# KumarRobotics/top_down_renderer

Measured on AMD Instinct MI355X. Metric: particle-updates/sec (render+score+resample), higher is better.
Workload: dtype f32

## Files before the change

include/tdr.h:

```cpp
#ifndef TDR_H_
#define TDR_H_

#include <stddef.h>
#include <stdint.h>

#ifdef __cplusplus
extern "C" {
#endif

#define TDR_OK 0
#define TDR_ERR_ARG (-1)
#define TDR_ERR_HIP (-2)
#define TDR_ERR_NOMEM (-3)

#define TDR_MAX_CLASSES 15
#define TDR_ST_FIELDS 7
enum { TDR_ST_INIT_X = 0, TDR_ST_INIT_Y = 1, TDR_ST_DX = 2, TDR_ST_DY = 3, TDR_ST_THETA = 4, TDR_ST_SCALE = 5,
       TDR_ST_HAVE_INIT = 6 };

typedef struct tdr_state {
  float init_x_px, init_y_px, dx_m, dy_m, theta, scale;
  uint8_t have_init;
  uint8_t pad_[3];
} tdr_state;
// ... 190 lines not shown
int tdr_config_compact(int on);
int tdr_config_shift_uniform(int mode);
float tdr_config_shift_uniform_span(float cells);
int tdr_config_ray_split(int k);
int tdr_config_cart_skip(int on);
int tdr_config_init_mfma(int on);
int tdr_config_uw_waves(int on);
int64_t tdr_shift_uniform_launches(void);

int tdr_profile_enable(int on);
int tdr_profile_score_ms(double* total_ms, int64_t* launches);
int tdr_profile_shares(double* dense_ms, double* scattered_ms, int64_t* scattered_particles);
int tdr_profile_variants(int64_t out[16]);

int64_t tdr_config_tuning(const char* name, int64_t value);
int tdr_selftest_score(void);
int tdr_k_selftest_round(const float* x, int64_t n, float limit, int32_t* out, void* stream);
int tdr_libm_variant(void);
int tdr_libm_force_variant(int variant);
int tdr_sincosf_host(const float* x, int64_t n, int variant, float* sin_out, float* cos_out);
int tdr_k_selftest_sincos(const float* x, int64_t n, float* sin_out, float* cos_out, void* stream);
int tdr_logf_host(const float* x, int64_t n, float* out);
int tdr_k_selftest_logf(const float* x, int64_t n, float* out, void* stream);
int tdr_k_selftest_atan2(const float* y, const float* x, int64_t n, float* out, void* stream);

int tdr_k_states_aos_to_soa(const tdr_state* aos, int64_t n, float* st, int64_t cap, void* stream);
int tdr_k_states_soa_to_aos(const float* st, int64_t cap, int64_t n, tdr_state* aos, void* stream);
size_t tdr_locality_tmp_ints(int64_t n, int map_rows, int map_cols);
int tdr_k_locality_order(const float* st, int64_t cap, int64_t n, int map_rows, int map_cols, int32_t* perm_out,
                         int32_t* keys_tmp, void* stream);
// ... 162 lines not shown
```

top_down_renderer_amd/_lib.py:

```python
import ctypes as C
import os

_PKG = os.path.dirname(os.path.abspath(__file__))
SO_PATH = os.environ.get("TDR_LIB_PATH") or os.path.join(_PKG, "libtdr_hip.so")

TDR_ST_FIELDS = 7
TDR_MAX_CLASSES = 15
TDR_SVG_NO_KEY = 0xFFFFFFFF


class FilterParamsC(C.Structure):
    _fields_ = [
        ("pos_cov", C.c_float), ("theta_cov", C.c_float), ("regularization", C.c_float),
        ("init_pos_px_x", C.c_float), ("init_pos_px_y", C.c_float), ("init_pos_px_cov", C.c_float),
        ("init_pos_m_x", C.c_float), ("init_pos_m_y", C.c_float),
        ("init_pos_deg_theta", C.c_float), ("init_pos_deg_cov", C.c_float),
        ("force_on_map", C.c_int32),
        ("fixed_scale", C.c_float), ("scale_log_min", C.c_float), ("scale_log_max", C.c_float),
        ("num_classes", C.c_int32),
        ("class_weights", C.c_float * 16),
    ]


class MapDescC(C.Structure):
# ... 96 lines not shown
    "tdr_rng_pipe_from_host": (_i, [_vp, _vp, _vp]),
    "tdr_rng_pipe_to_host": (_i, [_vp, _vp, _vp]),
    "tdr_rng_pipe_normals": (_i, [_vp, _i64, _i64, _i64, _i, C.POINTER(_vp), _vp]),
    "tdr_rng_pipe_uniform": (_i, [_vp, C.POINTER(_vp), _vp]),
    "tdr_rng_dev_workspace_bytes": (C.c_size_t, [_i64]),
    "tdr_k_rng_propagate_normals": (_i, [_vp, _i64, _i64, _i64, _i, _vp, _vp, _vp]),
    "tdr_k_rng_uniform": (_i, [_vp, _vp, _vp]),
    "tdr_rng_get_state_host": (_i, [_vp, _vp]),
    "tdr_rng_set_state_host": (_i, [_vp, _vp]),
    "tdr_k_resample_dev": (_i, [_vp, _i64, _i64, _vp, _i64, _i64, _vp, _vp]),
    "tdr_score_ctx_create": (_i, [C.POINTER(_vp)]),
    "tdr_score_ctx_destroy": (None, [_vp]),
    "tdr_score_ctx_span": (C.c_float, [_vp]),
    "tdr_score_ctx_trial_calls": (_i64, [_vp]),
    "tdr_config_tuning": (_i64, [C.c_char_p, _i64]),
    "tdr_selftest_score": (_i, []),
    "tdr_profile_variants": (_i, [C.POINTER(_i64)]),
    "tdr_score_ctx_set_polar_factors": (_i, [_vp, _vp, _i, _i]),
    "tdr_polar_factors_host": (_i, [_i, _i, _f, _f, _vp]),
    "tdr_k_score_polar_ctx": (_i, [C.POINTER(MapDescC), _vp, _vp, _i, _i, _f, C.POINTER(FilterParamsC), _vp, _i64, _i64,
                                   _i64, _vp, _f, _i, _vp, _vp, _vp, _vp]),
    "tdr_score_geo_workspace_floats": (C.c_size_t, [_i, _i, _i, _i64, _i64]),
    "tdr_k_score_polar_geo": (_i, [C.POINTER(MapDescC), C.POINTER(MapDescC), _vp, _vp, _vp, _f, _f, _i, _i, _f,
                                   C.POINTER(FilterParamsC), _vp, _i64, _i64, _i64, _vp, _f, _i, _vp, _vp, _vp]),
    "tdr_score_cart_workspace_floats": (C.c_size_t, [_i, _i, _i, _i64, _i64]),
    "tdr_k_score_cart": (_i, [C.POINTER(MapDescC), _vp, _i, _i, _f, C.POINTER(FilterParamsC), _vp, _i64, _i64, _i64,
                              _vp, _vp, _vp, _vp]),
    "tdr_score_cart_init_workspace_floats": (C.c_size_t, [_i, _i, _i, _i64, _i64]),
    "tdr_k_score_cart_init": (_i, [C.POINTER(MapDescC), _vp, _i, _i, _f, C.POINTER(FilterParamsC), _vp, _i64, _i64, _i64,
                                   _vp, _vp]),
# ... 141 lines not shown
```

top_down_renderer_amd/csrc/tdr_score.hip:

```cpp

#include "tdr_common.h"
#include "tdr_batch.h"
#include "tdr_sincosf.h"

struct ScoreArgs {
  const float* rec;
  int rows, cols;
  float resolution;
  const float* tab;
  const float* utab = nullptr;
  const float* scan_pk;
  int nb, nr;
  float res;
  const float* st;
  int64_t cap, n;
  const int32_t* order;
  const int32_t* count = nullptr;
  const int32_t* slot_base = nullptr;
  int use_theta_override = 0;
  float theta_override = 0.f;
  int only_uninit = 0;
  int group, nchunks;
  int64_t npad;
  float* part;
  const uint32_t* crec = nullptr;
  const float* dict = nullptr;
  int dict_n = 0;
  int ctiles_r = 0;
  unsigned kmask_off = 0;
  int kmask_row = 0;
  const int32_t* run_if = nullptr;
};

#include "tdr_score_dev.h"
#include "tdr_score_init.h"
#include "tdr_score_su.h"
#include "tdr_score_cart.h"


#ifdef TDR_SCORE_TIMELINE
#define TDR_TL_MAX (1 << 17)
__device__ unsigned long long g_timeline[2 * TDR_TL_MAX];
extern "C" int tdr_debug_read_timeline(unsigned long long* out, int n) {
  return hipMemcpyFromSymbol(out, HIP_SYMBOL(g_timeline), sizeof(unsigned long long) * 2 * (size_t)n) == hipSuccess ? 0 : -1;
}
#endif
template <int NV4, int U, bool KSLOT, bool USCALE, bool COMPACT, bool WIDE = false>
__device__ __forceinline__ void score_polar_body(const ScoreArgs& a, const unsigned bx, const unsigned by) {
  constexpr int RF = 4 * NV4;
  static_assert(!WIDE || (COMPACT && NV4 == 2), "wide compact records: 8-float dense records only");
  constexpr int CW = WIDE ? 4 : CmapShape<RF, KSLOT>::CW, LC = WIDE ? 1 : CmapShape<RF, KSLOT>::LC;
  constexpr int NDICT = WIDE ? TDR_CMAP_WIDE_MAX_DICT : TDR_CMAP_MAX_DICT;
#ifdef TDR_SCORE_TIMELINE
  const unsigned tl_id = blockIdx.y * gridDim.x + blockIdx.x;
  if (threadIdx.x == 0 && tl_id < TDR_TL_MAX) g_timeline[2 * tl_id] = wall_clock64();
#endif
  extern __shared__ float4 ring[];
  __shared__ float ldict[COMPACT ? NDICT : 1];
  const int lane = threadIdx.x & 63, wave = threadIdx.x >> 6;
  const int64_t slot = ((int64_t)bx * 4 + wave) * 64 + lane;
  if (a.run_if && !int_form_off(a.run_if)) return;
  const int64_t nact = a.count ? (int64_t)*a.count : a.n;
  if ((int64_t)bx * 256 >= nact) return;
  const bool valid = slot < nact;
  const int64_t sbase = a.slot_base ? (int64_t)*a.slot_base : 0;
  const int64_t p = a.order ? (int64_t)a.order[sbase + (valid ? slot : 0)] : (valid ? slot : 0);
  if (a.only_uninit && !__syncthreads_or(valid && a.st[TDR_ST_HAVE_INIT * a.cap + p] == 0.f)) return;
  const float scale = a.st[TDR_ST_SCALE * a.cap + p];
  const float cx = a.st[TDR_ST_DX * a.cap + p] * scale + a.st[TDR_ST_INIT_X * a.cap + p];
  const float cy = a.st[TDR_ST_DY * a.cap + p] * scale + a.st[TDR_ST_INIT_Y * a.cap + p];
  const float off0 = cy / a.resolution;
// ... 142 lines not shown
          int row = ic + shift;
          row -= row >= nb ? nb : 0;
          boff[u] = cell_offset(tab_at((int64_t)(j0 + jj) * nb + ic));
          sp[u] = rj + __mul24(row, rs);
        }
        step(std::false_type{}, boff, sp, min(U, nb - i));
      }
    }
  }
  if (sbase + slot < a.npad) {
    float* o = a.part + (int64_t)by * (RF + 1) * a.npad + sbase + slot;
#pragma unroll
    for (int k = 0; k < RF; k++) o[(int64_t)k * a.npad] = acc[k];
    o[(int64_t)RF * a.npad] = KSLOT ? acc[RF - 2] : known;
  }
#ifdef TDR_SCORE_TIMELINE
  __syncthreads();
  if (threadIdx.x == 0 && tl_id < TDR_TL_MAX) g_timeline[2 * tl_id + 1] = wall_clock64();
#endif
}
template <int NV4, int U, bool KSLOT, bool USCALE, bool COMPACT, bool WIDE = false>
__global__ __launch_bounds__(256, COMPACT ? (WIDE ? 3 : 5) : 1) void score_polar_kernel(ScoreArgs a) {
#if TDR_XCD_SWIZZLE
  const unsigned nbx = gridDim.x, per = (nbx + 7) / 8;
  unsigned bx = (blockIdx.x % 8) * per + blockIdx.x / 8;
  if (nbx % 8 != 0) bx = blockIdx.x;
#else
  const unsigned bx = blockIdx.x;
#endif
  score_polar_body<NV4, U, KSLOT, USCALE, COMPACT, WIDE>(a, bx, blockIdx.y);
}
template <int NV4, int U, bool KSLOT, bool USCALE, bool COMPACT, bool WIDE = false>
__global__ __launch_bounds__(256, COMPACT ? (WIDE ? 3 : 5) : 1) void score_polar_batch_kernel(const ScoreArgs* __restrict__ args,
                                                                                              const int32_t* __restrict__ blk, int k) {
// ... 396 lines not shown
#define TDR_CART_WAVE_MUL 2
static int64_t g_score_waves = 131072;
static int g_score_group = 0;
static int g_su_group = 0;
static int64_t score_wave_target() { return g_score_waves; }
extern "C" int tdr_config_init_ahead(int);
extern "C" int tdr_config_batch_init_search(int);
extern "C" int tdr_config_prefix_head(int);
extern "C" int tdr_config_ray_block_major(int);
extern "C" int tdr_config_ray_patch(int);
extern "C" int tdr_config_ray_borrow(int);
extern "C" int tdr_config_cart_seg_rows(int);
extern "C" int tdr_config_mt_stretches(int);
extern "C" int tdr_config_su_wave_span(int);
extern "C" int tdr_config_su_lds_pad(int);
extern "C" int tdr_config_init_device(int);
extern "C" int64_t tdr_config_init_window_words(int64_t);
extern "C" int64_t tdr_config_cart_init_chunk(int64_t);
extern "C" int64_t tdr_config_tuning(const char* name, int64_t value) {
  if (!name) return -1;
  const std::string n(name);
  if (n == "score_waves") { if (value > 0) g_score_waves = value; return g_score_waves; }
  if (n == "score_group") { if (value >= 0) g_score_group = (int)value; return g_score_group; }
  if (n == "su_group") { if (value >= 0) g_su_group = (int)value; return g_su_group; }
  if (n == "batch_init_search") return tdr_config_batch_init_search((int)std::max<int64_t>(value, -1));
  if (n == "init_ahead") return tdr_config_init_ahead((int)std::min<int64_t>(std::max<int64_t>(value, -1), 3));
  if (n == "prefix_head") return tdr_config_prefix_head((int)std::max<int64_t>(value, -1));
  if (n == "ray_borrow") return tdr_config_ray_borrow((int)std::max<int64_t>(value, -1));
  if (n == "ray_patch") return tdr_config_ray_patch((int)std::max<int64_t>(value, -1));
  if (n == "ray_block_major") return tdr_config_ray_block_major((int)std::max<int64_t>(value, -1));
  if (n == "cart_seg_rows") return tdr_config_cart_seg_rows((int)std::max<int64_t>(value, -1));
  if (n == "mt_stretches") return tdr_config_mt_stretches((int)std::max<int64_t>(value, -1));
  if (n == "su_lds_pad") return tdr_config_su_lds_pad((int)std::max<int64_t>(value, -1));
  if (n == "su_wave_span") return tdr_config_su_wave_span((int)std::max<int64_t>(value, -1));
  if (n == "init_device") return tdr_config_init_device((int)std::max<int64_t>(value, -1));
  if (n == "init_window_words") return tdr_config_init_window_words(value > 0 ? value : -1);
  if (n == "cart_init_chunk") return tdr_config_cart_init_chunk(value > 0 ? value : -1);
  return -1;
}
static void choose_chunks(int64_t n, int nr, int& rpc, int& nchunks, int target_mul = 1) {
  int64_t nbatches = cdiv(std::max<int64_t>(n, 1), 64);
  int64_t want = std::max<int64_t>(1, cdiv(score_wave_target() * target_mul, nbatches));
  nchunks = (int)std::min<int64_t>(nr, want);
  rpc = (int)cdiv(nr, nchunks);
  nchunks = (int)cdiv(nr, rpc);
}

__global__ void utab_kernel(const float* __restrict__ tab, int64_t n2, float scale, float res,
// ... 5 lines not shown
static int score_group_rings(int nb, int nr, int rf, int64_t n_total) {
  const int forced = g_score_group;
  const int64_t ring_bytes = std::max<int64_t>((int64_t)nb * rf * 4, 1);
  int g = (int)std::min<int64_t>(8, (32 * 1024) / ring_bytes);
  const int64_t chunks_wanted = cdiv(2048, cdiv(std::max<int64_t>(n_total, 1), 256));
  g = (int)std::min<int64_t>(g, std::max<int64_t>(1, nr / std::max<int64_t>(chunks_wanted, 1)));
  if (forced > 0) g = forced;
  g = std::max(1, std::min<int>(g, (int)((60 * 1024) / ring_bytes)));
  if (g >= TDR_SCORE_U) g -= g % TDR_SCORE_U;
  return std::max(g, 1);
}
extern "C" int tdr_cmap_words(int ncls);
struct ScoreWs {
  int group, nchunks;
  int su_group, su_nchunks;
  int64_t npad, npad_part, off_aux, off_utab, off_su, total;
  bool su;
  SuWs suw;
};
static ScoreWs score_ws(int ncls, int nb, int nr, int64_t n, int64_t n_total) {
  ScoreWs w;
  const int rf = tdr_rec_floats(ncls);
  if (n_total <= 0) n_total = n;
  w.group = score_group_rings(nb, nr, rf, n_total);
  if (w.group % 4 != 0 && tdr_cmap_words(ncls) != 0 && tdr_su_shape_ok(nb, nr, 4, n_total))
    w.group = std::max(4, w.group - w.group % 4);
  w.nchunks = (int)cdiv(nr, w.group);
  w.npad = cdiv(std::max<int64_t>(n, 1), 64) * 64;
  w.su = tdr_su_shape_ok(nb, nr, w.group, n_total) && tdr_cmap_words(ncls) != 0;
  w.su_group = w.group;
  {
    const int forced = g_su_group;
    if (w.su && w.group == 4 && nr % 8 == 0 && cdiv(n_total, 256) * (nr / 8) >= 4096) w.su_group = 8;
    if (w.su && forced >= 4 && forced % 4 == 0) w.su_group = forced;
  }
  w.su_nchunks = (int)cdiv(nr, w.su_group);
  w.npad_part = w.su ? su_npad(std::max<int64_t>(n, 1), nb) : w.npad;
  w.off_aux = w.su ? (int64_t)std::max(std::max(w.nchunks, w.su_nchunks), TDR_RAY_MAX_SPLIT) * std::max(rf + 1, 2 * ncls + 2) * w.npad_part
                   : (int64_t)w.nchunks * (rf + 1) * w.npad_part;
  w.off_utab = w.off_aux + 3 * w.npad + 64;
  w.off_su = (w.off_utab + 2 * (int64_t)nb * nr + 63) / 64 * 64;
  w.total = w.off_su;
  if (w.su) {
    w.suw = tdr_su_ws(nb, nr, w.su_group, std::max<int64_t>(n, 1));
    w.total += w.suw.total;
  }
  return w;
}
extern "C" size_t tdr_score_workspace_floats(int ncls, int nb, int nr, int64_t n, int64_t n_total) {
  if (ncls < 1 || ncls > TDR_MAX_CLASSES || nb < 1 || nr < 1 || n < 0) return 0;
  return (size_t)score_ws(ncls, nb, nr, n, n_total).total;
}
static int fill_utab(ScoreArgs& a, float* workspace, const ScoreWs& W, float uniform_scale, hipStream_t s) {
// ... 405 lines not shown
  a.part = workspace;
  int rc = fill_utab(a, workspace, W, uniform_scale, s);
  if (rc) return rc;
  float* res_flag = workspace + W.off_aux;
  if (init_search)
    if ((rc = tdr_score_init_search(map, a.tab, a.utab, scan_pk, nb, nr, res, fp, st, cap, n, n_total, perm, res_flag, a.npad, s)))
      return rc;
  FinalizeArgs f = make_finalize_args(map, fp, a.part, a.nchunks, a.npad, (int64_t)nb * nr, st, cap, n, perm, raw_w);
  if (int_form_applies(W, map, rf)) {
    const int32_t* slots = nullptr;
    const int32_t* counts = nullptr;
    SuLaunch L;
    L.map = map; L.tab = a.utab ? a.utab : a.tab; L.uniform_scale = a.utab != nullptr; L.scan_pk = scan_pk;
    L.nb = nb; L.nr = nr; L.rf = rf; L.res = res; L.st = st; L.cap = cap; L.n = n; L.perm = perm;
    L.group = W.su_group; L.nchunks = W.su_nchunks; L.npad = W.npad_part; L.part = a.part;
    L.fac = ctx && ctx->fac && ctx->fac_nb == nb && ctx->fac_nr == nr ? ctx->fac : nullptr;
    L.uscale = uniform_scale;
    L.wave_span = tdr_su_wave_span();
    L.ray_split = tdr_ray_splits(nb, nr, n, tdr_ray_block_major(L));
    L.ws = reinterpret_cast<int32_t*>(workspace + W.off_su);
    TunerScope tuner_scope(ctx, s);
    L.span = tdr_su_span_begin(ctx ? &ctx->tuner : nullptr,
                               ((int64_t)n << 24) ^ ((int64_t)nb << 12) ^ nr ^ ((int64_t)map->rows << 40), s);
    if ((rc = tdr_su_prepare(L, W.suw, s, &slots, &counts))) return rc;
    if ((rc = tdr_ray_prepare(L, W.suw, s))) return rc;
    const int32_t* inexact = counts + 4;
    {
      ScoreProfScope prof(s);
      {
        ShareProfScope sp(0, s, true);
        if ((rc = tdr_ray_score(L, W.suw, s))) return rc;
      }
      {
        ShareProfScope sp(1, s, true);
        if ((rc = tdr_su_score(L, W.suw, s))) return rc;
      }
      if (g_prof_on) { g_share_valid = true; g_share_counts = counts; }
      ScoreArgs r = a;
      r.run_if = inexact;
      if ((rc = launch_score(r, map, rf, s, false))) return rc;
    }
    launch_finalize_exact(f, map, W.npad_part, slots, counts, inexact, W.su_nchunks, L.ray_split, s);
    LAUNCH_CHECK("score_finalize_exact");
    launch_finalize(f, n, s);
  } else {
    if ((rc = launch_score(a, map, rf, s))) return rc;
    launch_finalize(f, n, s);
  }
  LAUNCH_CHECK("score_finalize");
  if (init_search) return tdr_score_init_fixup(res_flag, n, fp->regularization, raw_w, s);
  return TDR_OK;
}

__global__ void init_from_best_kernel(const float* __restrict__ best_cost, const float* __restrict__ best_theta,
                                      const int32_t* __restrict__ order, int64_t n, float* __restrict__ st, int64_t cap,
                                      GateArgs gate, float* __restrict__ res_flag) {
  const int64_t slot = (int64_t)blockIdx.x * blockDim.x + threadIdx.x;
// ... 166 lines not shown
```

top_down_renderer_amd/csrc/tdr_score_dev.h:

```cpp
#ifndef TDR_SCORE_DEV_H_
#define TDR_SCORE_DEV_H_
#include "tdr_common.h"

__device__ __forceinline__ int rot_shift_dev(float rot, int nb) {
  int s = (int)round((double)(rot * (float)nb / 2) / M_PI);
  s %= nb;
  if (s < 0) s += nb;
  return s;
}

__device__ __forceinline__ int round_half_away_clamped(float x) {
  const float y = x + 0.49999997f;
  int r;
  asm("v_cvt_flr_i32_f32 %0, %1" : "=v"(r) : "v"(y));
  return r;
}

template <int RF, bool KSLOT>
struct CmapShape {
  static constexpr int ND = KSLOT ? RF - 2 : RF - 1;
  static constexpr int CW = (ND + 2) / 3 <= 1 ? 1 : ((ND + 2) / 3 == 2 ? 2 : 4);
  static constexpr int LC = CW == 1 ? 3 : (CW == 2 ? 2 : 1);
};
template <int CW, int LC>
// ... 83 lines not shown
}

template <int RF, bool KSLOT>
__device__ __forceinline__ void cmap_decode_wide(const uint32_t (&w)[4], const float* ldict, float (&m)[RF]) {
  constexpr int ND = CmapShape<RF, KSLOT>::ND;
  static_assert(ND <= 7, "wide records hold up to seven distances");
#pragma unroll
  for (int k = 0; k < ND; k++) {
    const uint32_t boff = (k & 1) ? (w[k / 2] >> 16) : (w[k / 2] & 0xFFFCu);
    m[k] = *reinterpret_cast<const float*>(reinterpret_cast<const char*>(ldict) + boff);
  }
  const float kf = (float)(w[3] & 1u);
  if (KSLOT) m[RF - 2] = kf;
  m[RF - 1] = kf;
}
#endif
```

top_down_renderer_amd/csrc/tdr_score_ray.hip:

```cpp
#include "tdr_score_dev.h"
#include "tdr_score_su.h"

#define RAY_PR 16
#define RAY_PG 16
#define RAY_PATCH_MAX_NB 256
static bool g_ray_borrow = true;
extern "C" int tdr_config_ray_borrow(int on) {
  if (on >= 0) g_ray_borrow = on != 0;
  return g_ray_borrow ? 1 : 0;
}
static bool g_ray_patch = true;
extern "C" int tdr_config_ray_patch(int on) {
  if (on >= 0) g_ray_patch = on != 0;
  return g_ray_patch ? 1 : 0;
}
static bool g_ray_bm = true;
extern "C" int tdr_config_ray_block_major(int on) {
  if (on >= 0) g_ray_bm = on != 0;
  return g_ray_bm ? 1 : 0;
}
static inline bool ray_bm(const SuLaunch& L) { return g_ray_bm && L.fac != nullptr; }
static inline bool ray_patch(const SuLaunch& L) { return ray_bm(L) && g_ray_patch && L.nb % RAY_PG == 0 && L.nb <= RAY_PATCH_MAX_NB; }
static inline int ray_gq(int nr, bool bm) { return bm ? 1 : (nr <= 64 ? 1 : (nr <= 128 ? 2 : 4)); }
static inline int ray_blocks(int nr, bool bm) { return (int)cdiv(nr, 64 * ray_gq(nr, bm)); }
// ... 348 lines not shown
    if (lane == 0) {
      o[(int64_t)(2 * c) * a.npad] = (uint32_t)s;
      o[(int64_t)(2 * c + 1) * a.npad] = (uint32_t)(s >> 32);
    }
  }
#pragma unroll
  for (int dlt = 32; dlt > 0; dlt >>= 1) {
    known += __shfl_xor(known, dlt, 64);
    norm += __shfl_xor(norm, dlt, 64);
  }
  if (lane == 0) {
    o[(int64_t)(2 * a.ncls) * a.npad] = norm;
    o[(int64_t)(2 * a.ncls + 1) * a.npad] = known;
  }
}
template <int GQ, bool USCALE, bool BM = false, bool PATCH = false>
__global__ __launch_bounds__(256) void score_polar_ray_kernel(RayArgs a) {
  extern __shared__ unsigned long long lacc[];
  __shared__ uint32_t ldict[TDR_CMAP_MAX_DICT];
  __shared__ uint4 lut[16];
  __shared__ float2 ldir[PATCH ? RAY_PATCH_MAX_NB : 1];
  if (int_form_off(a.inexact)) return;
  if (a.fac && a.inexact[2] == 0) ray_body<GQ, USCALE, true, BM, PATCH>(a, lacc, ldict, lut, ldir);
  else ray_body<GQ, USCALE, false, BM, PATCH>(a, lacc, ldict, lut, ldir);
}


extern "C" size_t tdr_cmap_plane_offset_words(int ncls, int rows, int cols);
extern "C" size_t tdr_cmap_plane_words(int ncls, int rows, int cols);

bool tdr_ray_map_ok(const tdr_map_desc* map) {
  return map->crec && map->dict && map->cwords == tdr_cmap_words(map->ncls) && map->dict_n > 0 &&
         map->dict_n <= TDR_CMAP_MAX_DICT && tdr_cmap_plane_words(map->ncls, map->rows, map->cols) != 0;
}
static int g_ray_split = 0;
extern "C" int tdr_config_ray_split(int k) {
  if (k >= 0) g_ray_split = k > TDR_RAY_MAX_SPLIT ? TDR_RAY_MAX_SPLIT : k;
  return g_ray_split;
}
// ... 80 lines not shown
```

top_down_renderer_amd/csrc/tdr_score_su.h:

```cpp
#ifndef TDR_SCORE_SU_H_
#define TDR_SCORE_SU_H_
#include "tdr_common.h"

static inline int64_t su_npad(int64_t n, int nb) { return cdiv(n + 63 * std::min<int64_t>(nb, n), 64) * 64; }
bool tdr_su_shape_ok(int nb, int nr, int group, int64_t n_total);
struct SuWs {
  int64_t tab_su, desc, bbox, keys_in, keys_out, vals_in, vals_out, ints, slots, sort_tmp, ray_tab, ray_desc, ray_multi, ray_rad, total;
  int64_t slots2, wave_tmp;
};
#define TDR_SU_TAIL_INTS 10
#define TDR_RAY_MAX_SPLIT 8
SuWs tdr_su_ws(int nb, int nr, int group, int64_t n);

struct SuLaunch {
  const tdr_map_desc* map;
  const float* tab;
  bool uniform_scale;
  const float* scan_pk;
  int nb, nr, rf;
  float res;
  const float* st;
  int64_t cap, n;
  const int32_t* perm;
  int group, nchunks;
  int64_t npad;
  float* part;
  int ray_split;
  const float* fac;
  float uscale;
  int32_t* ws;
  float span;
  float wave_span = 0.f;
};
int tdr_su_prepare(const SuLaunch& L, const SuWs& W, hipStream_t s, const int32_t** slots_out, const int32_t** counts_out);
int tdr_su_order(const SuLaunch& L, const SuWs& W, hipStream_t s, const int32_t** slots_out, const int32_t** counts_out);
struct SpanTuner {
  int64_t shape = -1;
  int phase = -2;
  int settled_launches = 0;
// ... 19 lines not shown
```

top_down_renderer_amd/csrc/tdr_score_su.hip:

```cpp
#include <rocprim/device/device_radix_sort.hpp>

#include <atomic>

#include "tdr_score_dev.h"
#include "tdr_score_su.h"
#include "tdr_score_su_asm.h"

#define SU_CODE_FULL 0xFFu
#define SU_CODE_FULL_ALL 0xFEu
#define SU_CODE_PAD 0xFDu
#define SU_NSECT 8
#define SU_BOX_WORDS 4096

struct SuArgs {
  const uint32_t* crec;
  const uint32_t* kmask;
  int kcolw;
  unsigned kmask_off;
  const uint32_t* dict_int;
  int dict_n, ctiles_r;
  int pkcol;
  const int32_t* inexact;
  int rows, cols;
  float resolution;
  const float* tab_su;
  const uint32_t* desc;
  const float* bbox;
  const float* scan_pk;
  int nb, nr;
  float res;
  const float* st;
  int64_t cap;
  const int32_t* slots;
  const int32_t* nslots;
  int group, nchunks, ncls;
  int64_t npad;
  uint32_t* part;
  uint32_t* stats;
};

__global__ __launch_bounds__(256) void su_prep_kernel(const float* __restrict__ tab, const float* __restrict__ scan_pk,
                                                      int nb, int nr, int rf, int ncls, int ckconst, unsigned pbase,
                                                      unsigned plane_bytes, int group, int nchunks,
                                                      const float* __restrict__ dict, int dict_n, float* __restrict__ tab_su,
                                                      uint32_t* __restrict__ desc) {
  const int64_t t = (int64_t)blockIdx.x * blockDim.x + threadIdx.x;
  bool bad = false;
  for (int k = threadIdx.x; k < dict_n; k += blockDim.x) bad |= !(fabsf(dict[k]) <= 3.402823466e+38f);
  const bool dict_bad = __syncthreads_or(bad);
  const int64_t total = (int64_t)nchunks * nb * group;
// ... 228 lines not shown
    const int rank = __popcll(valid & (((uint64_t)1 << (t & 63)) - 1));
    out[(int64_t)counts[0] + oc1 + moved[w] + rank] = p;
  }
}
__global__ void su_copy_slots_kernel(const int32_t* __restrict__ src, const int32_t* __restrict__ counts, int32_t* __restrict__ dst) {
  const int64_t t = (int64_t)blockIdx.x * blockDim.x + threadIdx.x;
  if (t < (int64_t)counts[2]) dst[t] = src[t];
}

struct SuLds {
  uint32_t dict[TDR_CMAP_MAX_DICT];
  uint32_t bits[SU_BOX_WORDS];
  int box[4];
};

template <int NV4, bool KSLOT, bool USCALE>
__global__ __launch_bounds__(256) __attribute__((amdgpu_waves_per_eu(6, 8))) void score_polar_su_kernel(SuArgs a) {
  constexpr int RF = 4 * NV4;
  constexpr int ND = CmapShape<RF, KSLOT>::ND, CW = CmapShape<RF, KSLOT>::CW;
  constexpr bool ASM_LOOP = CW == 2 && ND == 6;
  __shared__ SuLds lds;
  if (int_form_off(a.inexact)) return;
  for (int t = threadIdx.x; t < a.dict_n; t += 256) lds.dict[t] = a.dict_int[t];
  const int lane = threadIdx.x & 63, wave = __builtin_amdgcn_readfirstlane(threadIdx.x >> 6);
  const int64_t nsl = (int64_t)__builtin_amdgcn_readfirstlane(*a.nslots);
  if ((int64_t)blockIdx.x * 256 >= nsl) return;
  const int64_t base = ((int64_t)blockIdx.x * 4 + wave) * 64;
  const bool active = base < nsl;
  const int32_t sp = active ? a.slots[base + lane] : -1;
  const int32_t p0 = a.slots[active ? base : (int64_t)blockIdx.x * 256];
  const int64_t p = sp >= 0 ? sp : p0;
  const float scale = a.st[TDR_ST_SCALE * a.cap + p];
  const float cx = a.st[TDR_ST_DX * a.cap + p] * scale + a.st[TDR_ST_INIT_X * a.cap + p];
  const float cy = a.st[TDR_ST_DY * a.cap + p] * scale + a.st[TDR_ST_INIT_Y * a.cap + p];
  const float off0 = cy / a.resolution;
  const float off1 = cx / a.resolution;
  const int shift = __builtin_amdgcn_readfirstlane(rot_shift_dev(a.st[TDR_ST_THETA * a.cap + p], a.nb));
  const int nb = a.nb, G = a.group;
  const int j0 = blockIdx.y * G, gn = min(a.nr - j0, G);
  const float rmaxf = (float)a.rows, cmaxf = (float)a.cols;
  const int ckcol = a.ctiles_r * 128 - 16 * CW;
  const int pkcol = a.pkcol;
  const uint32_t ckconst = (uint32_t)(a.ctiles_r * 128 + 128);
  auto su_rec_const = [&](uint32_t cd) -> uint32_t {
    return cd != 0 && cd < SU_CODE_PAD ? ckconst + 4u * (((cd - 1u) * 11u) >> 5) : ckconst;
  };
  typedef const float __attribute__((address_space(4))) * tdr_const_f;
  typedef const uint32_t __attribute__((address_space(4))) * tdr_const_u;
  const tdr_const_f tbase = (tdr_const_f)a.tab_su + (int64_t)blockIdx.y * nb * G * 2;
  const tdr_const_u dbase = (tdr_const_u)a.desc + (int64_t)blockIdx.y * nb * G * 4;
  const tdr_const_f bbase = (tdr_const_f)a.bbox + (int64_t)blockIdx.y * SU_NSECT * 4;
  const tdr_const_f scanc = (tdr_const_f)a.scan_pk;
  const uint32_t* __restrict__ crec = a.crec;
  const uint32_t* __restrict__ kmask = a.kmask;
  const unsigned lds_base = (unsigned)(uintptr_t)&lds;
  const unsigned lbits_lds = (unsigned)(uintptr_t)&lds.bits[0];

  typedef float tdr_v2f __attribute__((ext_vector_type(2)));
  const tdr_v2f offv = {off0, off1};
  typedef const uint32_t __attribute__((address_space(3))) * tdr_lds_u;
  auto lds_word = [](unsigned byte_addr) -> uint32_t { return *reinterpret_cast<tdr_lds_u>((uintptr_t)byte_addr); };
  const char* __restrict__ crecb = reinterpret_cast<const char*>(a.crec);
  auto map_dword = [&](unsigned off) -> uint32_t { return *reinterpret_cast<const uint32_t*>(crecb + off); };
  auto map_ushort = [&](unsigned off) -> uint32_t { return *reinterpret_cast<const uint16_t*>(crecb + off); };
  const bool weird = !(fabsf(off0) <= 1e9f) || !(fabsf(off1) <= 1e9f) || (!USCALE && !(fabsf(scale * a.res) <= 1e9f));
  auto field = [&](const uint32_t (&w)[CW], int k) -> uint32_t {
// ... 312 lines not shown
          nleft = __builtin_amdgcn_readfirstlane(nleft); wleft = __builtin_amdgcn_readfirstlane(wleft);
        }
        return;
      }
    }
    for (int i = i0; i < i1; i++) {
      int r = i + shift;
      r -= r >= nb ? nb : 0;
      for (int jj = 0; jj < gn; jj += 4) {
        if (dbase[((int64_t)r * G + jj) * 4 + 3] >> 31) cpp_step(i, r, jj, krow4, kconst);
        else cpp_step_plane(i, r, jj, krow4, kconst);
      }
    }
  };

  for (int sect = 0; sect < SU_NSECT; sect++) {
    const int i0 = (int)((int64_t)sect * nb / SU_NSECT), i1 = (int)((int64_t)(sect + 1) * nb / SU_NSECT);
    float a0 = bbase[4 * sect], b0 = bbase[4 * sect + 1], a1 = bbase[4 * sect + 2], b1 = bbase[4 * sect + 3];
    if constexpr (!USCALE) {
      const float x0 = (a0 * scale) * a.res, y0 = (b0 * scale) * a.res, x1 = (a1 * scale) * a.res, y1 = (b1 * scale) * a.res;
      a0 = fminf(x0, y0); b0 = fmaxf(x0, y0); a1 = fminf(x1, y1); b1 = fmaxf(x1, y1);
    }
    int rl = (int)fminf(fmaxf(floorf(a0 + off0) - 1.f, -1.f), rmaxf), rh = (int)fminf(fmaxf(ceilf(b0 + off0) + 1.f, -1.f), rmaxf);
    int cl = (int)fminf(fmaxf(floorf(a1 + off1) - 1.f, -1.f), cmaxf), ch = (int)fminf(fmaxf(ceilf(b1 + off1) + 1.f, -1.f), cmaxf);
    if (weird) { rl = -1; rh = a.rows; cl = -1; ch = a.cols; }
    if (!active) { rl = 0x7FFFFFFF; rh = -0x7FFFFFFF; cl = 0x7FFFFFFF; ch = -0x7FFFFFFF; }
#pragma unroll
    for (int d = 32; d > 0; d >>= 1) {
      rl = min(rl, __shfl_xor(rl, d)); rh = max(rh, __shfl_xor(rh, d));
      cl = min(cl, __shfl_xor(cl, d)); ch = max(ch, __shfl_xor(ch, d));
    }
// ... 60 lines not shown
      else far_sector(i0, i1);
    }
  }
  if (active) {
    const int64_t slot = base + lane;
    uint32_t* o = a.part + (int64_t)blockIdx.y * (2 * a.ncls + 2) * a.npad + slot;
#pragma unroll
    for (int k = 0; k < ND; k++)
      if (k < a.ncls) {
        o[(int64_t)(2 * k) * a.npad] = (uint32_t)acc[k];
        o[(int64_t)(2 * k + 1) * a.npad] = (uint32_t)(acc[k] >> 32);
      }
    o[(int64_t)(2 * a.ncls) * a.npad] = norm;
    o[(int64_t)(2 * a.ncls + 1) * a.npad] = known;
  }
}

static int g_su_mode = 1;
extern "C" int tdr_config_shift_uniform(int mode) {
  if (mode >= 0) g_su_mode = mode > 2 ? 2 : mode;
  return g_su_mode;
}
extern "C" size_t tdr_cmap_tile_words(int ncls, int rows, int cols);
extern "C" size_t tdr_cmap_plane_offset_words(int ncls, int rows, int cols);
extern "C" size_t tdr_cmap_plane_words(int ncls, int rows, int cols);
#define SU_SPAN_START 16.f
static bool g_su_span_fixed = false;
static float g_su_span = SU_SPAN_START;
extern "C" float tdr_config_shift_uniform_span(float cells) {
  if (cells >= 0.f) { g_su_span = cells; g_su_span_fixed = true; }
// ... 45 lines not shown
}
float tdr_su_wave_span() { return g_su_wave_span; }
static int g_su_lds_pad = 0;
extern "C" int tdr_config_su_lds_pad(int bytes) {
  if (bytes >= 0) g_su_lds_pad = bytes;
  return g_su_lds_pad;
}
static std::atomic<int64_t> g_su_launches{0};
extern "C" int64_t tdr_shift_uniform_launches(void) { return g_su_launches.load(); }
bool tdr_su_shape_ok(int nb, int nr, int group, int64_t n_total) {
  if (g_su_mode == 0) return false;
  if (group % 4 != 0 || nb > 4095) return false;
  if (g_su_mode == 2) return true;
  if ((int64_t)nb * nr < 8192) return false;
  return n_total >= (int64_t)64 * nb;
}
static size_t su_sort_tmp_bytes(int64_t n) {
  size_t bytes = 0;
  uint32_t* k = nullptr;
  int32_t* v = nullptr;
  hipError_t e = rocprim::radix_sort_pairs(nullptr, bytes, k, k, v, v, (size_t)std::max<int64_t>(n, 1), 0u, 12u,
                                           (hipStream_t)0, false);
  if (e != hipSuccess || bytes == 0) bytes = (size_t)(n + 4096) * 16;
  return bytes;
}
SuWs tdr_su_ws(int nb, int nr, int group, int64_t n) {
  SuWs w;
  const int64_t nchunks = cdiv(nr, group), nbins = nchunks * nb * group;
  int64_t o = 0;
  auto take = [&](int64_t words) { const int64_t at = o; o += (words + 63) / 64 * 64; return at; };
// ... 93 lines not shown
  const int lc = map->cwords == 1 ? 3 : (map->cwords == 2 ? 2 : 1);
  u.crec = map->crec; u.dict_int = reinterpret_cast<const uint32_t*>(map->dict) + TDR_CMAP_MAX_DICT;
  u.dict_n = map->dict_n; u.ctiles_r = (map->rows >> lc) + 2;
  u.pkcol = plane_trows(map->rows) * 128 - 16;
  u.inexact = nslots + 4;
  u.rows = map->rows; u.cols = map->cols; u.resolution = map->resolution;
  u.tab_su = reinterpret_cast<const float*>(base + W.tab_su);
  u.desc = reinterpret_cast<const uint32_t*>(base + W.desc);
  u.bbox = reinterpret_cast<const float*>(base + W.bbox);
  u.kmask = map->crec + tdr_cmap_tile_words(map->ncls, map->rows, map->cols);
  u.kcolw = kmask_trows(map->rows) * 32;
  u.kmask_off = (unsigned)(tdr_cmap_tile_words(map->ncls, map->rows, map->cols) * 4);
  u.scan_pk = L.scan_pk;
  u.nb = L.nb; u.nr = L.nr; u.res = L.res; u.st = L.st; u.cap = L.cap;
  u.slots = base + W.slots; u.nslots = nslots;
  u.group = L.group; u.nchunks = L.nchunks; u.ncls = map->ncls; u.npad = L.npad; u.part = reinterpret_cast<uint32_t*>(L.part);
  u.stats = tdr_profile_stats_ptr();
  const dim3 grid((unsigned)cdiv(L.npad, 256), (unsigned)L.nchunks), block(256);
  const bool ks = tdr_has_kslot(map->ncls, L.rf), us = L.uniform_scale;
#define TDR_LAUNCH_SU(NV4)                                                                         \
  if (ks && us) hipLaunchKernelGGL((score_polar_su_kernel<NV4, true, true>), grid, block, g_su_lds_pad, s, u);  \
  else if (ks) hipLaunchKernelGGL((score_polar_su_kernel<NV4, true, false>), grid, block, g_su_lds_pad, s, u);  \
  else if (us) hipLaunchKernelGGL((score_polar_su_kernel<NV4, false, true>), grid, block, g_su_lds_pad, s, u);  \
  else hipLaunchKernelGGL((score_polar_su_kernel<NV4, false, false>), grid, block, g_su_lds_pad, s, u);
  switch (L.rf / 4) {
    case 1: TDR_LAUNCH_SU(1) break;
    case 2: TDR_LAUNCH_SU(2) break;
    case 3: TDR_LAUNCH_SU(3) break;
    default: return fail(TDR_ERR_ARG, "score: no shift-uniform kernel for record size %d", L.rf);
  }
#undef TDR_LAUNCH_SU
  LAUNCH_CHECK("score_polar_su");
  g_su_launches.fetch_add(1);
// ... 3 lines not shown
```

Before: 22.40 million.

## Split trailing shift-uniform row groups into sector partitions to balance grid tail

```diff
diff --git a/include/tdr.h b/include/tdr.h
--- a/include/tdr.h
+++ b/include/tdr.h
@@ -228,6 +228,7 @@
 int tdr_profile_variants(int64_t out[16]);
 
 int64_t tdr_config_tuning(const char* name, int64_t value);
+int tdr_su_tail_plan(int nchunks, int k, int q, int row, int* group, int* s0, int* s1);
 int tdr_selftest_score(void);
 int tdr_k_selftest_round(const float* x, int64_t n, float limit, int32_t* out, void* stream);
 int tdr_libm_variant(void);
diff --git a/top_down_renderer_amd/_lib.py b/top_down_renderer_amd/_lib.py
--- a/top_down_renderer_amd/_lib.py
+++ b/top_down_renderer_amd/_lib.py
@@ -134,6 +134,7 @@
     "tdr_score_ctx_span": (C.c_float, [_vp]),
     "tdr_score_ctx_trial_calls": (_i64, [_vp]),
     "tdr_config_tuning": (_i64, [C.c_char_p, _i64]),
+    "tdr_su_tail_plan": (_i, [_i, _i, _i, _i, C.POINTER(_i), C.POINTER(_i), C.POINTER(_i)]),
     "tdr_selftest_score": (_i, []),
     "tdr_profile_variants": (_i, [C.POINTER(_i64)]),
     "tdr_score_ctx_set_polar_factors": (_i, [_vp, _vp, _i, _i]),
diff --git a/top_down_renderer_amd/csrc/tdr_score.hip b/top_down_renderer_amd/csrc/tdr_score.hip
--- a/top_down_renderer_amd/csrc/tdr_score.hip
+++ b/top_down_renderer_amd/csrc/tdr_score.hip
@@ -38,23 +38,14 @@
 #include "tdr_score_cart.h"
 
 
-#ifdef TDR_SCORE_TIMELINE
-#define TDR_TL_MAX (1 << 17)
-__device__ unsigned long long g_timeline[2 * TDR_TL_MAX];
-extern "C" int tdr_debug_read_timeline(unsigned long long* out, int n) {
-  return hipMemcpyFromSymbol(out, HIP_SYMBOL(g_timeline), sizeof(unsigned long long) * 2 * (size_t)n) == hipSuccess ? 0 : -1;
-}
-#endif
+TDR_TL_BUFFER(g_timeline, tdr_debug_read_timeline)
 template <int NV4, int U, bool KSLOT, bool USCALE, bool COMPACT, bool WIDE = false>
 __device__ __forceinline__ void score_polar_body(const ScoreArgs& a, const unsigned bx, const unsigned by) {
   constexpr int RF = 4 * NV4;
   static_assert(!WIDE || (COMPACT && NV4 == 2), "wide compact records: 8-float dense records only");
   constexpr int CW = WIDE ? 4 : CmapShape<RF, KSLOT>::CW, LC = WIDE ? 1 : CmapShape<RF, KSLOT>::LC;
   constexpr int NDICT = WIDE ? TDR_CMAP_WIDE_MAX_DICT : TDR_CMAP_MAX_DICT;
-#ifdef TDR_SCORE_TIMELINE
-  const unsigned tl_id = blockIdx.y * gridDim.x + blockIdx.x;
-  if (threadIdx.x == 0 && tl_id < TDR_TL_MAX) g_timeline[2 * tl_id] = wall_clock64();
-#endif
+  TDR_TL_BEGIN(g_timeline)
   extern __shared__ float4 ring[];
   __shared__ float ldict[COMPACT ? NDICT : 1];
   const int lane = threadIdx.x & 63, wave = threadIdx.x >> 6;
@@ -227,10 +218,7 @@
     for (int k = 0; k < RF; k++) o[(int64_t)k * a.npad] = acc[k];
     o[(int64_t)RF * a.npad] = KSLOT ? acc[RF - 2] : known;
   }
-#ifdef TDR_SCORE_TIMELINE
-  __syncthreads();
-  if (threadIdx.x == 0 && tl_id < TDR_TL_MAX) g_timeline[2 * tl_id + 1] = wall_clock64();
-#endif
+  TDR_TL_END(g_timeline)
 }
 template <int NV4, int U, bool KSLOT, bool USCALE, bool COMPACT, bool WIDE = false>
 __global__ __launch_bounds__(256, COMPACT ? (WIDE ? 3 : 5) : 1) void score_polar_kernel(ScoreArgs a) {
@@ -657,6 +645,8 @@
 extern "C" int tdr_config_mt_stretches(int);
 extern "C" int tdr_config_su_wave_span(int);
 extern "C" int tdr_config_su_lds_pad(int);
+extern "C" int tdr_config_su_tail_groups(int);
+extern "C" int tdr_config_su_tail_parts(int);
 extern "C" int tdr_config_init_device(int);
 extern "C" int64_t tdr_config_init_window_words(int64_t);
 extern "C" int64_t tdr_config_cart_init_chunk(int64_t);
@@ -675,6 +665,8 @@
   if (n == "cart_seg_rows") return tdr_config_cart_seg_rows((int)std::max<int64_t>(value, -1));
   if (n == "mt_stretches") return tdr_config_mt_stretches((int)std::max<int64_t>(value, -1));
   if (n == "su_lds_pad") return tdr_config_su_lds_pad((int)std::max<int64_t>(value, -1));
+  if (n == "su_tail_groups") return tdr_config_su_tail_groups((int)std::min<int64_t>(std::max<int64_t>(value, -1), 1 << 20));
+  if (n == "su_tail_parts") return tdr_config_su_tail_parts((int)std::min<int64_t>(std::max<int64_t>(value, -1), 8));
   if (n == "su_wave_span") return tdr_config_su_wave_span((int)std::max<int64_t>(value, -1));
   if (n == "init_device") return tdr_config_init_device((int)std::max<int64_t>(value, -1));
   if (n == "init_window_words") return tdr_config_init_window_words(value > 0 ? value : -1);
@@ -710,6 +702,7 @@
 struct ScoreWs {
   int group, nchunks;
   int su_group, su_nchunks;
+  int su_tail_k, su_tail_q, su_rows;
   int64_t npad, npad_part, off_aux, off_utab, off_su, total;
   bool su;
   SuWs suw;
@@ -728,11 +721,20 @@
   {
     const int forced = g_su_group;
     if (w.su && w.group == 4 && nr % 8 == 0 && cdiv(n_total, 256) * (nr / 8) >= 4096) w.su_group = 8;
+    int k16 = 0, q16 = 1;
+    if (w.su && w.su_group == 8 && nr % 16 == 0 && cdiv(std::max<int64_t>(n, 1), 256) * (nr / 16) >= 4096)
+      tdr_su_tail(nr / 16, std::max<int64_t>(n, 1), &k16, &q16);
+    if (k16 > 0) w.su_group = 16;
     if (w.su && forced >= 4 && forced % 4 == 0) w.su_group = forced;
   }
   w.su_nchunks = (int)cdiv(nr, w.su_group);
+  tdr_su_tail(w.su_nchunks, std::max<int64_t>(n, 1), &w.su_tail_k, &w.su_tail_q);
+  {
+    int g, s0, s1;
+    w.su_rows = su_tail_plan(w.su_nchunks, w.su_tail_k, w.su_tail_q, -1, &g, &s0, &s1);
+  }
   w.npad_part = w.su ? su_npad(std::max<int64_t>(n, 1), nb) : w.npad;
-  w.off_aux = w.su ? (int64_t)std::max(std::max(w.nchunks, w.su_nchunks), TDR_RAY_MAX_SPLIT) * std::max(rf + 1, 2 * ncls + 2) * w.npad_part
+  w.off_aux = w.su ? (int64_t)std::max(std::max(w.nchunks, w.su_rows), TDR_RAY_MAX_SPLIT) * std::max(rf + 1, 2 * ncls + 2) * w.npad_part
                    : (int64_t)w.nchunks * (rf + 1) * w.npad_part;
   w.off_utab = w.off_aux + 3 * w.npad + 64;
   w.off_su = (w.off_utab + 2 * (int64_t)nb * nr + 63) / 64 * 64;
@@ -1168,6 +1170,7 @@
     L.map = map; L.tab = a.utab ? a.utab : a.tab; L.uniform_scale = a.utab != nullptr; L.scan_pk = scan_pk;
     L.nb = nb; L.nr = nr; L.rf = rf; L.res = res; L.st = st; L.cap = cap; L.n = n; L.perm = perm;
     L.group = W.su_group; L.nchunks = W.su_nchunks; L.npad = W.npad_part; L.part = a.part;
+    L.tail_k = W.su_tail_k; L.tail_q = W.su_tail_q; L.rows = W.su_rows;
     L.fac = ctx && ctx->fac && ctx->fac_nb == nb && ctx->fac_nr == nr ? ctx->fac : nullptr;
     L.uscale = uniform_scale;
     L.wave_span = tdr_su_wave_span();
@@ -1194,7 +1197,7 @@
       r.run_if = inexact;
       if ((rc = launch_score(r, map, rf, s, false))) return rc;
     }
-    launch_finalize_exact(f, map, W.npad_part, slots, counts, inexact, W.su_nchunks, L.ray_split, s);
+    launch_finalize_exact(f, map, W.npad_part, slots, counts, inexact, W.su_rows, L.ray_split, s);
     LAUNCH_CHECK("score_finalize_exact");
     launch_finalize(f, n, s);
   } else {
diff --git a/top_down_renderer_amd/csrc/tdr_score_dev.h b/top_down_renderer_amd/csrc/tdr_score_dev.h
--- a/top_down_renderer_amd/csrc/tdr_score_dev.h
+++ b/top_down_renderer_amd/csrc/tdr_score_dev.h
@@ -121,4 +121,26 @@
   if (KSLOT) m[RF - 2] = kf;
   m[RF - 1] = kf;
 }
+#ifdef TDR_SCORE_TIMELINE
+#define TDR_TL_MAX (1 << 17)
+#define TDR_TL_BUFFER(BUF, READER)                                                                                       \
+  __device__ unsigned long long BUF[2 * TDR_TL_MAX];                                                                     \
+  extern "C" int READER(unsigned long long* out, int n) {                                                                \
+    void* dev = nullptr;                                                                                                 \
+    if (n < 0 || n > TDR_TL_MAX || hipDeviceSynchronize() != hipSuccess) return -1;                                      \
+    if (hipMemcpyFromSymbol(out, HIP_SYMBOL(BUF), sizeof(unsigned long long) * 2 * (size_t)n) != hipSuccess) return -1;  \
+    if (hipGetSymbolAddress(&dev, HIP_SYMBOL(BUF)) != hipSuccess) return -1;                                             \
+    return hipMemset(dev, 0, sizeof(unsigned long long) * 2 * TDR_TL_MAX) == hipSuccess ? 0 : -1;                        \
+  }
+#define TDR_TL_BEGIN(BUF)                                                                                                \
+  const unsigned tl_id = blockIdx.y * gridDim.x + blockIdx.x;                                                            \
+  if (threadIdx.x == 0 && tl_id < TDR_TL_MAX) BUF[2 * tl_id] = wall_clock64();
+#define TDR_TL_END(BUF)                                                                                                  \
+  __syncthreads();                                                                                                       \
+  if (threadIdx.x == 0 && tl_id < TDR_TL_MAX) BUF[2 * tl_id + 1] = wall_clock64();
+#else
+#define TDR_TL_BUFFER(BUF, READER)
+#define TDR_TL_BEGIN(BUF)
+#define TDR_TL_END(BUF)
 #endif
+#endif
diff --git a/top_down_renderer_amd/csrc/tdr_score_ray.hip b/top_down_renderer_amd/csrc/tdr_score_ray.hip
--- a/top_down_renderer_amd/csrc/tdr_score_ray.hip
+++ b/top_down_renderer_amd/csrc/tdr_score_ray.hip
@@ -386,6 +386,7 @@
     o[(int64_t)(2 * a.ncls + 1) * a.npad] = known;
   }
 }
+TDR_TL_BUFFER(g_timeline_ray, tdr_debug_read_timeline_ray)
 template <int GQ, bool USCALE, bool BM = false, bool PATCH = false>
 __global__ __launch_bounds__(256) void score_polar_ray_kernel(RayArgs a) {
   extern __shared__ unsigned long long lacc[];
@@ -393,8 +394,13 @@
   __shared__ uint4 lut[16];
   __shared__ float2 ldir[PATCH ? RAY_PATCH_MAX_NB : 1];
   if (int_form_off(a.inexact)) return;
+#ifdef TDR_SCORE_TIMELINE
+  if ((int64_t)blockIdx.x * 4 >= (int64_t)a.counts[1] * a.nsplit) return;
+#endif
+  TDR_TL_BEGIN(g_timeline_ray)
   if (a.fac && a.inexact[2] == 0) ray_body<GQ, USCALE, true, BM, PATCH>(a, lacc, ldict, lut, ldir);
   else ray_body<GQ, USCALE, false, BM, PATCH>(a, lacc, ldict, lut, ldir);
+  TDR_TL_END(g_timeline_ray)
 }
 
 
diff --git a/top_down_renderer_amd/csrc/tdr_score_su.h b/top_down_renderer_amd/csrc/tdr_score_su.h
--- a/top_down_renderer_amd/csrc/tdr_score_su.h
+++ b/top_down_renderer_amd/csrc/tdr_score_su.h
@@ -12,6 +12,24 @@
 #define TDR_RAY_MAX_SPLIT 8
 SuWs tdr_su_ws(int nb, int nr, int group, int64_t n);
 
+#define TDR_SU_NSECT 8
+__host__ __device__ static inline int su_tail_plan(int nchunks, int k, int q, int row, int* group, int* s0, int* s1) {
+  const int lq = q >= 8 ? 3 : (q >= 4 ? 2 : (q >= 2 ? 1 : 0));
+  const int kk = k < 0 ? 0 : (k > nchunks ? nchunks : k);
+  const int head = nchunks - kk, rows = head + (kk << lq);
+  if (row < 0 || row >= rows) return rows;
+  if (row < head) {
+    *group = row; *s0 = 0; *s1 = TDR_SU_NSECT;
+  } else {
+    const int t = row - head, part = t & ((1 << lq) - 1);
+    *group = head + (t >> lq);
+    *s0 = part << (3 - lq);
+    *s1 = (part + 1) << (3 - lq);
+  }
+  return rows;
+}
+void tdr_su_tail(int nchunks, int64_t n, int* k, int* q);
+
 struct SuLaunch {
   const tdr_map_desc* map;
   const float* tab;
@@ -23,6 +41,8 @@
   int64_t cap, n;
   const int32_t* perm;
   int group, nchunks;
+  int tail_k = 0, tail_q = 1;
+  int rows = 0;
   int64_t npad;
   float* part;
   int ray_split;
diff --git a/top_down_renderer_amd/csrc/tdr_score_su.hip b/top_down_renderer_amd/csrc/tdr_score_su.hip
--- a/top_down_renderer_amd/csrc/tdr_score_su.hip
+++ b/top_down_renderer_amd/csrc/tdr_score_su.hip
@@ -9,7 +9,7 @@
 #define SU_CODE_FULL 0xFFu
 #define SU_CODE_FULL_ALL 0xFEu
 #define SU_CODE_PAD 0xFDu
-#define SU_NSECT 8
+#define SU_NSECT TDR_SU_NSECT
 #define SU_BOX_WORDS 4096
 
 struct SuArgs {
@@ -34,6 +34,7 @@
   const int32_t* slots;
   const int32_t* nslots;
   int group, nchunks, ncls;
+  int tail_k, tail_q;
   int64_t npad;
   uint32_t* part;
   uint32_t* stats;
@@ -292,6 +293,7 @@
   int box[4];
 };
 
+TDR_TL_BUFFER(g_timeline_su, tdr_debug_read_timeline_su)
 template <int NV4, bool KSLOT, bool USCALE>
 __global__ __launch_bounds__(256) __attribute__((amdgpu_waves_per_eu(6, 8))) void score_polar_su_kernel(SuArgs a) {
   constexpr int RF = 4 * NV4;
@@ -303,6 +305,7 @@
   const int lane = threadIdx.x & 63, wave = __builtin_amdgcn_readfirstlane(threadIdx.x >> 6);
   const int64_t nsl = (int64_t)__builtin_amdgcn_readfirstlane(*a.nslots);
   if ((int64_t)blockIdx.x * 256 >= nsl) return;
+  TDR_TL_BEGIN(g_timeline_su)
   const int64_t base = ((int64_t)blockIdx.x * 4 + wave) * 64;
   const bool active = base < nsl;
   const int32_t sp = active ? a.slots[base + lane] : -1;
@@ -315,7 +318,9 @@
   const float off1 = cx / a.resolution;
   const int shift = __builtin_amdgcn_readfirstlane(rot_shift_dev(a.st[TDR_ST_THETA * a.cap + p], a.nb));
   const int nb = a.nb, G = a.group;
-  const int j0 = blockIdx.y * G, gn = min(a.nr - j0, G);
+  int rgroup = 0, sect0 = 0, sect1 = SU_NSECT;
+  su_tail_plan(a.nchunks, a.tail_k, a.tail_q, (int)blockIdx.y, &rgroup, &sect0, &sect1);
+  const int j0 = rgroup * G, gn = min(a.nr - j0, G);
   const float rmaxf = (float)a.rows, cmaxf = (float)a.cols;
   const int ckcol = a.ctiles_r * 128 - 16 * CW;
   const int pkcol = a.pkcol;
@@ -325,9 +330,9 @@
   };
   typedef const float __attribute__((address_space(4))) * tdr_const_f;
   typedef const uint32_t __attribute__((address_space(4))) * tdr_const_u;
-  const tdr_const_f tbase = (tdr_const_f)a.tab_su + (int64_t)blockIdx.y * nb * G * 2;
-  const tdr_const_u dbase = (tdr_const_u)a.desc + (int64_t)blockIdx.y * nb * G * 4;
-  const tdr_const_f bbase = (tdr_const_f)a.bbox + (int64_t)blockIdx.y * SU_NSECT * 4;
+  const tdr_const_f tbase = (tdr_const_f)a.tab_su + (int64_t)rgroup * nb * G * 2;
+  const tdr_const_u dbase = (tdr_const_u)a.desc + (int64_t)rgroup * nb * G * 4;
+  const tdr_const_f bbase = (tdr_const_f)a.bbox + (int64_t)rgroup * SU_NSECT * 4;
   const tdr_const_f scanc = (tdr_const_f)a.scan_pk;
   const uint32_t* __restrict__ crec = a.crec;
   const uint32_t* __restrict__ kmask = a.kmask;
@@ -670,7 +675,7 @@
     }
   };
 
-  for (int sect = 0; sect < SU_NSECT; sect++) {
+  for (int sect = sect0; sect < sect1; sect++) {
     const int i0 = (int)((int64_t)sect * nb / SU_NSECT), i1 = (int)((int64_t)(sect + 1) * nb / SU_NSECT);
     float a0 = bbase[4 * sect], b0 = bbase[4 * sect + 1], a1 = bbase[4 * sect + 2], b1 = bbase[4 * sect + 3];
     if constexpr (!USCALE) {
@@ -761,6 +766,7 @@
     o[(int64_t)(2 * a.ncls) * a.npad] = norm;
     o[(int64_t)(2 * a.ncls + 1) * a.npad] = known;
   }
+  TDR_TL_END(g_timeline_su)
 }
 
 static int g_su_mode = 1;
@@ -836,6 +842,31 @@
   if (g_su_mode == 2) return true;
   if ((int64_t)nb * nr < 8192) return false;
   return n_total >= (int64_t)64 * nb;
+}
+static int g_su_tail_groups = 4, g_su_tail_parts = 4;
+extern "C" int tdr_config_su_tail_groups(int k) {
+  if (k >= 0) g_su_tail_groups = k;
+  return g_su_tail_groups;
+}
+extern "C" int tdr_config_su_tail_parts(int q) {
+  if (q >= 0) g_su_tail_parts = q >= 8 ? 8 : (q >= 4 ? 4 : (q >= 2 ? 2 : 1));
+  return g_su_tail_parts;
+}
+void tdr_su_tail(int nchunks, int64_t n, int* k, int* q) {
+  *k = std::min(g_su_tail_groups, nchunks);
+  *q = g_su_tail_parts;
+  if (g_su_mode != 2 && cdiv(std::max<int64_t>(n, 1), 256) * nchunks < 2 * 256 * 6) *k = 0;
+  if (*k == 0 || *q == 1) { *k = 0; *q = 1; }
+}
+extern "C" int tdr_su_tail_plan(int nchunks, int k, int q, int row, int* group, int* s0, int* s1) {
+  int g = 0, a = 0, b = 0;
+  const int rows = su_tail_plan(nchunks, k, q, row, &g, &a, &b);
+  if (row >= 0 && row < rows) {
+    if (group) *group = g;
+    if (s0) *s0 = a;
+    if (s1) *s1 = b;
+  }
+  return rows;
 }
 static size_t su_sort_tmp_bytes(int64_t n) {
   size_t bytes = 0;
@@ -959,9 +990,12 @@
   u.scan_pk = L.scan_pk;
   u.nb = L.nb; u.nr = L.nr; u.res = L.res; u.st = L.st; u.cap = L.cap;
   u.slots = base + W.slots; u.nslots = nslots;
-  u.group = L.group; u.nchunks = L.nchunks; u.ncls = map->ncls; u.npad = L.npad; u.part = reinterpret_cast<uint32_t*>(L.part);
+  u.group = L.group; u.nchunks = L.nchunks; u.tail_k = L.tail_k; u.tail_q = L.tail_q; u.ncls = map->ncls; u.npad = L.npad; u.part = reinterpret_cast<uint32_t*>(L.part);
   u.stats = tdr_profile_stats_ptr();
-  const dim3 grid((unsigned)cdiv(L.npad, 256), (unsigned)L.nchunks), block(256);
+  int rg, r0, r1;
+  const int rows = su_tail_plan(L.nchunks, L.tail_k, L.tail_q, -1, &rg, &r0, &r1);
+  if (L.rows != rows) return fail(TDR_ERR_ARG, "score: %d rows of partial sums for a plan of %d", L.rows, rows);
+  const dim3 grid((unsigned)cdiv(L.npad, 256), (unsigned)rows), block(256);
   const bool ks = tdr_has_kslot(map->ncls, L.rf), us = L.uniform_scale;
 #define TDR_LAUNCH_SU(NV4)                                                                         \
   if (ks && us) hipLaunchKernelGGL((score_polar_su_kernel<NV4, true, true>), grid, block, g_su_lds_pad, s, u);  \
```

Result: faster. 23.09 million (median of 6 runs) (+3.1%).
